# ndoll1998/lightgrad

Hardware: AMD Instinct MI355X
Metric: mnist_mlp_train_steps_per_sec_batch1024_per_gpu (higher is better)
Workload: dtype f32; 1 GPU; mnist_mlp_784x512x10_bias_batch1024_mse_adabelief_lr1e-3 (fwd+bwd+allreduce+optimizer); batch_per_gpu=1024, global_batch=1024, parallelism=dp1, optimizer_kernel=fused, input_requires_grad=True, dispatch=hipGraph replay (python tape captured once; 13 consecutive steps per graph), steps_per_graph=13, device=AMD Instinct (gfx950), compute_units=256, clock_mhz=2400

## Files before the change

### lightgrad_amd/csrc/gemm.hip

```cpp
#include "common.h"
#include "gelu_common.h"
#include "adam_common.h"
#include "tail_jobs.h"
#include "mse_finalize.h"
#include "head_fwd_body.h"
#include <cstdlib>
#include <cstring>
#include <type_traits>

namespace lg {

typedef float f32x16 __attribute__((ext_vector_type(16)));
typedef unsigned int u32x4 __attribute__((ext_vector_type(4)));
typedef float f32x4 __attribute__((ext_vector_type(4)));

#ifndef LG_SMALL_PD
#define LG_SMALL_PD 2
#endif
constexpr int kSmallTilePrefetch = LG_SMALL_PD;
#ifndef LG_WAVE_PRIVATE_PD
#define LG_WAVE_PRIVATE_PD 1
#endif
constexpr int kWavePrivatePrefetch = LG_WAVE_PRIVATE_PD;

struct FastDiv {
    uint32_t m, s;
    __device__ __forceinline__ int div(int n) const { return int((uint64_t(uint32_t(n)) * m) >> s); }
};
static FastDiv make_fastdiv(int64_t d) {
    if (d < 1) d = 1;
    uint32_t l = 0;
    while ((int64_t(1) << l) < d) ++l;
    FastDiv f;
    f.m = uint32_t((uint64_t(1) << (31 + l)) / uint64_t(d) + 1);
    f.s = 31 + l;
    return f;
}

struct GemmArgs {
    const float* A;
    const float* B;
    float*       C;
    int64_t M, N, K;
    int64_t lda, ldb, ldc;
    int64_t sA, sB, sC;
    int64_t sA2, sB2, sC2;
    int     batch_inner;
    int     tiles_m, tiles_n;
    int     nwg;
    int     accumulate;
    const float* bias;
    const float* addend;
    int64_t      ldadd;
    int     group_m;
    int     k_slices;
    int64_t k_per_slice;
    float*  W;
    int*    tickets;
    float*  rowsum;
    int     rowsum_accumulate;
    FastDiv div_per_batch, div_slices, div_gspan, div_group, div_last_group, div_batch_inner;
    int     k_tail;
    short   relu_a, relu_b;
    int     act;
    float*  aux;
    int     multi;
    int64_t boff[3], coff[3], biasoff[3];
    int     seg_k, seg_steps;
    int64_t seg_jump[2];
    const AdamPlan* adam_c;
    const AdamPlan* adam_r;
#ifdef LG_GEMM_TIMELINE
    unsigned long long* tl;
#endif
};

// ... 52 lines not shown
    constexpr int BM = 64, BN = 32, BK = 32, WM = 2, WN = 1, KG = 2, XT = 0;
    constexpr bool AKC = true, BKC = true, VA = true, VB = true;
    __shared__ __attribute__((aligned(16))) float lds[gemm_lds_floats<BM, BN, BK, AKC, BKC, KG>()];
    if (int(blockIdx.x) < g.nwg) {
        int* const signal_tickets = c.tickets;
        const int signal_stride = c.stride, signal_per_row = c.per_row;
#define LG_TILE_OWNS_LDS 0
#define LG_TILE_BID int(blockIdx.x)
#undef LG_TILE_SIGNAL
#define LG_TILE_SIGNAL 1
#include "gemm_tile_body.inc"
#undef LG_TILE_SIGNAL
#undef LG_TILE_BID
#undef LG_TILE_OWNS_LDS
    } else {
        const HeadFwd& a = c.h;
        const int tid = threadIdx.x, lane = tid & 63, wave = tid >> 6;
        const int wn = a.outs * a.hidden;
        for (int i = tid * 4; i < wn; i += 1024) *reinterpret_cast<float4*>(lds + i) = *reinterpret_cast<const float4*>(a.w + i);
        const int64_t row0 = int64_t(int(blockIdx.x) - g.nwg) * 4;
        int* const ticket = c.tickets + int(row0 / BM) * c.stride;
        const int64_t block_rows = a.rows - (row0 / BM) * BM < BM ? a.rows - (row0 / BM) * BM : BM;
        const int readers = int((block_rows + 3) / 4);
        int* const flag = ticket + 16;
        int* const done = ticket + 17;
        __shared__ int seen;
        if (tid == 0) {
            int ok = 1;
            const unsigned long long t0 = wall_clock64();
            while (__hip_atomic_load(flag, __ATOMIC_RELAXED, __HIP_MEMORY_SCOPE_AGENT) == 0) {
                __builtin_amdgcn_s_sleep(2);
                if (wall_clock64() - t0 > 200000000ull) {
                    __hip_atomic_fetch_or(c.status, LG_STATUS_HANDOFF_TIMEOUT, __ATOMIC_RELAXED, __HIP_MEMORY_SCOPE_SYSTEM);
                    ok = 0;
                    break;
                }
            }
            seen = ok;
        }
        __syncthreads();
        __builtin_amdgcn_fence(__ATOMIC_ACQUIRE, "wavefront");
        const int64_t row = row0 + wave;
        if (row < a.rows) head_fwd_row<OMAX, true>(a, lds, row, lane);
        if (tid == 0 && seen) {
            if (__hip_atomic_fetch_add(done, 1, __ATOMIC_RELAXED, __HIP_MEMORY_SCOPE_AGENT) == readers - 1) {
                __hip_atomic_store(done, 0, __ATOMIC_RELAXED, __HIP_MEMORY_SCOPE_AGENT);
                __hip_atomic_store(flag, 0, __ATOMIC_RELAXED, __HIP_MEMORY_SCOPE_AGENT);
            }
        }
    }
}

template <int PD, bool SECOND_BKC = false>
__global__ void __launch_bounds__(256) sgemm_pair_wgrad_xgrad(GemmArgs first, GemmArgs second) {
    constexpr int L1 = gemm_lds_floats<64, 64, 32, false, false, 1>(), L2 = gemm_lds_floats<64, 64, 32, true, SECOND_BKC, 1>();
    __shared__ __attribute__((aligned(16))) float lds[L1 > L2 ? L1 : L2];
    constexpr int BM = 64, BN = 64, BK = 32, WM = 2, WN = 2, KG = 1, XT = 0;
    constexpr bool VA = true, VB = true;
#define LG_TILE_OWNS_LDS 0
    if (int(blockIdx.x) < first.nwg) {
        constexpr bool AKC = false, BKC = false;
        const GemmArgs& g = first;
#define LG_TILE_BID int(blockIdx.x)
#include "gemm_tile_body.inc"
#undef LG_TILE_BID
    } else {
        constexpr bool AKC = true, BKC = SECOND_BKC;
        const GemmArgs& g = second;
#define LG_TILE_BID (int(blockIdx.x) - first.nwg)
#include "gemm_tile_body.inc"
#undef LG_TILE_BID
    }
#undef LG_TILE_OWNS_LDS
}

int lg_mse_finalize_job(const float* row_loss, int64_t rows, float inv_n, float* loss);
struct PairFirsts { GemmArgs w[2]; };
struct LossJob {
    const float* row_loss;
    float*       loss;
    int64_t      rows;
    float        inv_n;
};
template <int PD>
__global__ void __launch_bounds__(256) sgemm_triple_wgrad2_xgrad(PairFirsts firsts, GemmArgs second, LossJob job) {
    constexpr int L1 = gemm_lds_floats<64, 64, 32, false, false, 1>(), L2 = gemm_lds_floats<64, 64, 32, true, false, 1>();
    __shared__ __attribute__((aligned(16))) float lds[L1 > L2 ? L1 : L2];
    constexpr int BM = 64, BN = 64, BK = 32, WM = 2, WN = 2, KG = 1, XT = 0;
    constexpr bool VA = true, VB = true;
#define LG_TILE_OWNS_LDS 0
    const int n0w = firsts.w[0].nwg, n1w = firsts.w[1].nwg;
    if (int(blockIdx.x) < n0w + n1w) {
        constexpr bool AKC = false, BKC = false;
        const int which = int(blockIdx.x) >= n0w ? 1 : 0;
        const GemmArgs g = firsts.w[which];
#define LG_TILE_BID (int(blockIdx.x) - (which ? n0w : 0))
#include "gemm_tile_body.inc"
#undef LG_TILE_BID
    } else if (int(blockIdx.x) < n0w + n1w + second.nwg) {
        constexpr bool AKC = true, BKC = false;
        const GemmArgs& g = second;
#define LG_TILE_BID (int(blockIdx.x) - n0w - n1w)
#include "gemm_tile_body.inc"
#undef LG_TILE_BID
    } else {
        finalize_loss(job.row_loss, job.rows, job.inv_n, job.loss, lds);
    }
#undef LG_TILE_OWNS_LDS
}

constexpr int kGroupMax = 14;
struct GroupProduct {
    const float* A;
    const float* B;
    float*       C;
    float*       W;
    int*         tickets;
    float*       rowsum;
    int64_t      M, N, K, lda, ldb, ldc, k_per_slice;
    int          tiles_m, tiles_n, nwg, accumulate, group_m, k_slices, rowsum_accumulate, k_tail;
    FastDiv      div_per_batch, div_slices, div_gspan, div_group, div_last_group, div_batch_inner;
};
static GroupProduct pack_product(const GemmArgs& g) {
    return GroupProduct{g.A, g.B, g.C, g.W, g.tickets, g.rowsum, g.M, g.N, g.K, g.lda, g.ldb, g.ldc, g.k_per_slice,
                        g.tiles_m, g.tiles_n, g.nwg, g.accumulate, g.group_m, g.k_slices, g.rowsum_accumulate, g.k_tail,
                        g.div_per_batch, g.div_slices, g.div_gspan, g.div_group, g.div_last_group, g.div_batch_inner};
}
__device__ __forceinline__ GemmArgs unpack_product(const GroupProduct& p) {
    GemmArgs g{};
    g.A = p.A; g.B = p.B; g.C = p.C; g.W = p.W; g.tickets = p.tickets; g.rowsum = p.rowsum;
    g.M = p.M; g.N = p.N; g.K = p.K; g.lda = p.lda; g.ldb = p.ldb; g.ldc = p.ldc; g.k_per_slice = p.k_per_slice;
    g.tiles_m = p.tiles_m; g.tiles_n = p.tiles_n; g.nwg = p.nwg; g.accumulate = p.accumulate; g.group_m = p.group_m;
    g.k_slices = p.k_slices; g.rowsum_accumulate = p.rowsum_accumulate; g.k_tail = p.k_tail;
    g.div_per_batch = p.div_per_batch; g.div_slices = p.div_slices; g.div_gspan = p.div_gspan; g.div_group = p.div_group;
    g.div_last_group = p.div_last_group; g.div_batch_inner = p.div_batch_inner;
    g.batch_inner = 1;
    return g;
}

struct GemmGroup {
    GroupProduct p[kGroupMax];
    int      first[kGroupMax + 1];
    int      count;
    const float* cs_in;
    float*       cs_out;
    int64_t      cs_rows, cs_cols, cs_ld;
    int          cs_accumulate, cs_wgs;
    int          tail_wgs;
    TailGroup    tail;
};

static_assert(sizeof(GemmGroup) <= 4096, "the group travels as kernel arguments");

template <int PD>
__global__ void __launch_bounds__(256) sgemm_group_wgrad(GemmGroup grp) {
    __shared__ __attribute__((aligned(16))) float lds[gemm_lds_floats<64, 64, 32, false, false, 1>()];
    constexpr int BM = 64, BN = 64, BK = 32, WM = 2, WN = 2, KG = 1, XT = 0;
    constexpr bool VA = true, VB = true, AKC = false, BKC = false;
    if (int(blockIdx.x) < grp.cs_wgs) {
        const int q = threadIdx.x >> 6, cl = threadIdx.x & 63;
// ... 14 lines not shown
            grp.cs_out[col] = grp.cs_accumulate ? grp.cs_out[col] + v : v;
        }
        return;
    }
    const int bid = int(blockIdx.x) - grp.cs_wgs;
    if (bid >= grp.first[grp.count]) {
        tail_group_body(grp.tail, bid - grp.first[grp.count]);
        return;
    }
    int which = 0;
    while (which + 1 < grp.count && bid >= grp.first[which + 1]) ++which;
    const GemmArgs g = unpack_product(grp.p[which]);
#define LG_TILE_OWNS_LDS 0
#define LG_TILE_BID (bid - grp.first[which])
#include "gemm_tile_body.inc"
#undef LG_TILE_BID
#undef LG_TILE_OWNS_LDS
}

static thread_local int32_t g_gemm_plan[8] = {-1, 0, 0, 0, 0, 0, 0, 0};

template <int BM, int BN, int BK, int WM, int WN, bool AKC, bool BKC, int KG>
static bool launch_layout(const GemmArgs& g, bool va, bool vb) {
    dim3 grid(g.nwg), block(WM * WN * KG * 64);
    hipStream_t s = rt().stream;
    constexpr int PD = (BM * BN <= 64 * 64) ? kSmallTilePrefetch : 2;
    static_assert(BM * BN < 256 * 256 || PD <= 2, "a third K-tile in flight does not fit the 256x256 tile's 128 registers: ring registers would spill while their loads are in flight");
    if constexpr (kWavePrivateTile<BM, BN, WM, WN, KG> && AKC && BKC) {
        static const char* kloop_env = getenv("LG_GEMM_KLOOP");
        if (va && vb && !(kloop_env && strcmp(kloop_env, "coop") == 0)) {
            constexpr int WPD = kWavePrivatePrefetch;
            if (g.multi) hipLaunchKernelGGL((sgemm_mfma<BM, BN, BK, WM, WN, true, true, true, true, WPD, KG, 1, true>), grid, block, 0, s, g);
            else         hipLaunchKernelGGL((sgemm_mfma<BM, BN, BK, WM, WN, true, true, true, true, WPD, KG, 0, true>), grid, block, 0, s, g);
            return true;
        }
    }
    if constexpr (kHasExtras<BM, BN>) {
        if constexpr (AKC && BKC)  { if (g.multi) { hipLaunchKernelGGL((sgemm_mfma<BM, BN, BK, WM, WN, AKC, BKC, true, true, PD, KG, 1>), grid, block, 0, s, g); return false; } }
        if constexpr (AKC && !BKC) { if (g.seg_k) { hipLaunchKernelGGL((sgemm_mfma<BM, BN, BK, WM, WN, AKC, BKC, true, true, PD, KG, 2>), grid, block, 0, s, g); return false; } }
    }
    if constexpr (!kHasExtras<BM, BN>) {
        hipLaunchKernelGGL((sgemm_mfma<BM, BN, BK, WM, WN, AKC, BKC, true, true, PD, KG>), grid, block, 0, s, g);
        return false;
    }
    if (va && vb)  hipLaunchKernelGGL((sgemm_mfma<BM, BN, BK, WM, WN, AKC, BKC, true, true, PD, KG>), grid, block, 0, s, g);
    else if (va)   hipLaunchKernelGGL((sgemm_mfma<BM, BN, BK, WM, WN, AKC, BKC, true, false, 1, KG>), grid, block, 0, s, g);
    else if (vb)   hipLaunchKernelGGL((sgemm_mfma<BM, BN, BK, WM, WN, AKC, BKC, false, true, 1, KG>), grid, block, 0, s, g);
    else           hipLaunchKernelGGL((sgemm_mfma<BM, BN, BK, WM, WN, AKC, BKC, false, false, 1, KG>), grid, block, 0, s, g);
    return false;
}

#ifdef LG_GEMM_TIMELINE
static void lg_debug_timeline_state(unsigned long long* buf, int nwg, int slices, int tiles);
#endif
struct PairState {
    int      active = 0;
    int      count = 0;
    bool     second_bkc = false;
    GemmArgs args[3];
    bool     is_s[3] = {false, false, false};
    int64_t  batch[3] = {1, 1, 1};
    int64_t  tiles = 0;
    LossJob  job{};
};
static PairState& pair_state() { static PairState p; return p; }

static void pair_launch_single(const GemmArgs& g, bool is_s) {
    dim3 grid(g.nwg), block(256);
    constexpr int PD = kSmallTilePrefetch;
    if (!is_s) hipLaunchKernelGGL((sgemm_mfma<64, 64, 32, 2, 2, false, false, true, true, PD, 1>), grid, block, 0, rt().stream, g);
    else if (pair_state().second_bkc) hipLaunchKernelGGL((sgemm_mfma<64, 64, 32, 2, 2, true, true, true, true, PD, 1>), grid, block, 0, rt().stream, g);
    else           hipLaunchKernelGGL((sgemm_mfma<64, 64, 32, 2, 2, true, false, true, true, PD, 1>), grid, block, 0, rt().stream, g);
}

static int pair_retune(GemmArgs& g, int64_t others_nwg) {
    const int64_t tiles = int64_t(g.tiles_m) * g.tiles_n;
    static const char* pair_slices_env = getenv("LG_GEMM_PAIR_SLICES");
    if (pair_slices_env || g.nwg != tiles * g.k_slices || g.seg_k || tiles >= 256 || g.K < 128) return LG_OK;
    constexpr int BK = 32, BM = 64, BN = 64;
    const double cus = rt().compute_units > 0 ? rt().compute_units : 256;
    const int64_t k_tiles = (g.K + BK - 1) / BK;
    int64_t best_sl = g.k_slices;
    double best = 1e30;
    for (int64_t sl = 1; sl <= 64 && (sl == 1 || sl * 2 <= k_tiles); ++sl) {
        const double per_cu = double(tiles * sl + others_nwg) / cus;
        const double c = per_cu > 1.0 ? double(int64_t(per_cu + 0.999)) : 1.0;
        const double cost = double((k_tiles + sl - 1) / sl) * (c <= 1.0 ? 0.68 : 0.43 * c + 0.17) + (sl > 1 ? 1.8 + 0.85 * double(sl) : 0.0);
        if (cost < best) { best = cost; best_sl = sl; }
    }
    int64_t k_per_slice = ((g.K + best_sl - 1) / best_sl + BK - 1) / BK * BK;
    best_sl = (g.K + k_per_slice - 1) / k_per_slice;
    if (best_sl == g.k_slices) return LG_OK;
    if (g.W) { const int rc = lg_free(g.W); g.W = nullptr; if (rc != LG_OK) return rc; }
    g.k_per_slice = k_per_slice;
    g.k_slices = int(best_sl);
    g.nwg = int(tiles * best_sl);
    g.div_slices = make_fastdiv(best_sl);
    if (best_sl > 1) {
        const int rc = lg_malloc(reinterpret_cast<void**>(&g.W), size_t(tiles * best_sl) * BM * BN * sizeof(float));
        if (rc != LG_OK) return rc;
    }
    return LG_OK;
}

static int pair_flush(bool keep_collecting) {
    PairState& P = pair_state();
    int rc = LG_OK;
    bool job_done = false;
    if (P.count == 3) {
        rc = pair_retune(P.args[1], int64_t(P.args[0].nwg) + P.args[2].nwg);
        if (rc != LG_OK) { P.count = 0; return rc; }
        PairFirsts firsts;
        firsts.w[0] = P.args[0];
        firsts.w[1] = P.args[1];
        const int spare = P.job.loss ? 1 : 0;
        hipLaunchKernelGGL((sgemm_triple_wgrad2_xgrad<kSmallTilePrefetch>), dim3(P.args[0].nwg + P.args[1].nwg + P.args[2].nwg + spare), dim3(256), 0,
                           rt().stream, firsts, P.args[2], P.job);
        job_done = true;
    } else if (P.count == 2 && P.is_s[1]) {
        rc = pair_retune(P.args[0], P.args[1].nwg);
        if (rc != LG_OK) { P.count = 0; return rc; }
#ifdef LG_GEMM_TIMELINE
        if (P.args[0].tl) {
            (void)hipMemsetAsync(P.args[0].tl, 0, size_t(P.args[0].nwg + P.args[1].nwg) * 64, rt().stream);
            lg_debug_timeline_state(P.args[0].tl, P.args[0].nwg + P.args[1].nwg, P.args[0].k_slices * 100 + P.args[1].k_slices, P.args[0].nwg);
        }
#endif
        if (P.second_bkc)
            hipLaunchKernelGGL((sgemm_pair_wgrad_xgrad<kSmallTilePrefetch, true>), dim3(P.args[0].nwg + P.args[1].nwg), dim3(256), 0, rt().stream,
                               P.args[0], P.args[1]);
        else
            hipLaunchKernelGGL((sgemm_pair_wgrad_xgrad<kSmallTilePrefetch, false>), dim3(P.args[0].nwg + P.args[1].nwg), dim3(256), 0, rt().stream,
                               P.args[0], P.args[1]);
    } else {
        for (int i = 0; i < P.count; ++i) pair_launch_single(P.args[i], P.is_s[i]);
    }
    for (int i = 0; i < P.count; ++i)
        if (P.args[i].W) { const int r = lg_free(P.args[i].W); if (r != LG_OK) rc = r; }
    P.count = 0;
    P.tiles = 0;
    if (job_done) P.job = LossJob{};
    if (!keep_collecting && P.active) P.active = 2;
    return rc;
}

struct WriteSpan { uintptr_t lo, hi; };
static WriteSpan product_c_span(const GemmArgs& g, int64_t batch) {
    const int64_t outer = batch / g.batch_inner;
    int64_t lo = 0, hi = (g.M - 1) * g.ldc + g.N;
    const int64_t reach[2] = {(outer - 1) * g.sC, int64_t(g.batch_inner - 1) * g.sC2};
    for (int64_t r : reach) { if (r < 0) lo += r; else hi += r; }
    const uintptr_t base = reinterpret_cast<uintptr_t>(g.C);
    return WriteSpan{base + uintptr_t(lo * 4), base + uintptr_t(hi * 4)};
}
static bool spans_meet(WriteSpan a, WriteSpan b) { return a.lo < b.hi && b.lo < a.hi; }
static bool products_write_alike(const GemmArgs& a, int64_t batch_a, const GemmArgs& b, int64_t batch_b) {
    const WriteSpan none{0, 0};
    const WriteSpan ca = product_c_span(a, batch_a), cb = product_c_span(b, batch_b);
    const WriteSpan ra = a.rowsum ? WriteSpan{reinterpret_cast<uintptr_t>(a.rowsum), reinterpret_cast<uintptr_t>(a.rowsum + a.M)} : none;
    const WriteSpan rb = b.rowsum ? WriteSpan{reinterpret_cast<uintptr_t>(b.rowsum), reinterpret_cast<uintptr_t>(b.rowsum + b.M)} : none;
    return spans_meet(ca, cb) || spans_meet(ca, rb) || spans_meet(ra, cb) || spans_meet(ra, rb);
}

static bool pair_try_defer(GemmArgs& g, bool akc, bool bkc, bool va, bool vb, int64_t batch) {
    PairState& P = pair_state();
    if (P.active != 1) return false;
    const int slot = P.count;
    for (int i = 0; i < slot; ++i)
        if (products_write_alike(P.args[i], P.batch[i], g, batch)) return false;
    const bool f_form = !akc && !bkc, s_form = akc;
    bool fits = slot < 3 && va && vb && batch >= 1;
    if (slot == 0)      fits = fits && f_form;
    else if (slot == 1) fits = fits && !P.is_s[0] && (f_form || s_form);
    else                fits = fits && !P.is_s[1] && s_form && !bkc && batch == 1 && !g.relu_a && !g.relu_b;
    if (slot == 1 && f_form) fits = fits && batch == 1 && P.args[0].nwg == int64_t(P.args[0].tiles_m) * P.args[0].tiles_n * P.args[0].k_slices;
    const int64_t tiles = int64_t(g.tiles_m) * g.tiles_n * batch;
    if (!fits || P.tiles + tiles > rt().n_tickets) return false;
    g.tickets = rt().tickets + P.tiles;
// ... 41 lines not shown
        bool ride = true;
        for (int i = 0; i < G.count; ++i) ride = ride && !ln_group_writes(G.queued[i].C) && !ln_group_writes(G.queued[i].rowsum);
        ride = ride && !ln_group_writes(G.grp.cs_wgs > 0 ? G.grp.cs_out : nullptr);
        G.grp.tail_wgs = 0;
        if (ride && tail_take(&G.grp.tail)) {
            G.grp.tail_wgs = G.grp.tail.first[G.grp.tail.ln.count + G.grp.tail.n_scatter];
        }
        hipLaunchKernelGGL((sgemm_group_wgrad<kSmallTilePrefetch>), dim3(G.grp.cs_wgs + G.grp.tail_wgs + G.grp.first[G.count]), dim3(256), 0, rt().stream, G.grp);
        if (G.grp.tail_wgs > 0) { const int r = tail_taken(); if (r != LG_OK) rc = r; }
    }
    for (int i = 0; i < G.count; ++i)
        if (G.queued[i].W) { const int r = lg_free(G.queued[i].W); if (r != LG_OK) rc = r; }
    G.count = 0;
    G.tiles = 0;
    G.grp.cs_wgs = 0;
    return rc;
}

static bool group_try_defer(GemmArgs& g, bool akc, bool bkc, bool va, bool vb, int64_t batch, int& rc) {
    GroupState& G = group_state();
    rc = LG_OK;
    if (G.active != 1 || pair_state().active) return false;
    const int64_t tiles = int64_t(g.tiles_m) * g.tiles_n;
    if (akc || bkc || !va || !vb || batch != 1 || tiles > kGroupTiles || g.relu_a || g.relu_b || g.multi || g.seg_k) return false;
    if (g.adam_c || g.adam_r) return false;
    bool clash = false;
    for (int i = 0; i < G.count; ++i)
        clash = clash || G.queued[i].C == g.C || (g.rowsum && G.queued[i].rowsum == g.rowsum);
    if (ln_group_writes(g.C) || ln_group_writes(g.rowsum)) {
        rc = gemm_group_flush_pending();
        if (rc != LG_OK) return false;
    } else if (clash || G.count == kGroupMax || G.tiles + tiles > tickets_group_end()) {
        rc = group_flush();
        if (rc != LG_OK) return false;
    }
    g.tickets = rt().tickets + G.tiles;
    G.tiles += tiles;
    G.queued[G.count] = g;
    G.count += 1;
    return true;
}

bool gemm_group_is_open() { return group_state().active == 1; }

int gemm_group_flush_pending() {
    if (pair_state().count) { const int prc = pair_flush(true); if (prc != LG_OK) return prc; }
    const int rc = group_flush();
    const int rc2 = ln_group_flush_pending();
    return rc != LG_OK ? rc : rc2;
}

#ifdef LG_GEMM_TIMELINE
static unsigned long long* g_tl_buf = nullptr;
static int g_tl_nwg = 0, g_tl_slices = 0, g_tl_tiles = 0;
static void lg_debug_timeline_state(unsigned long long* buf, int nwg, int slices, int tiles) {
    g_tl_buf = buf; g_tl_nwg = nwg; g_tl_slices = slices; g_tl_tiles = tiles;
}
#endif

template <int BM, int BN, int BK, int WM, int WN, int KG = 1>
static int launch_config(const GemmArgs& base, bool akc, bool bkc, bool va, bool vb, int64_t batch) {
    GemmArgs g = base;
    g.tiles_m = int((g.M + BM - 1) / BM);
    g.tiles_n = int((g.N + (g.rowsum ? 1 : 0) + BN - 1) / BN);
    const int64_t tiles = int64_t(g.tiles_m) * g.tiles_n * batch;
    int64_t slices = 1;
    if (kCanSplitK<BM, BN, KG> && tiles < 256 && g.K >= 4 * BK) {
        const double cus = rt().compute_units > 0 ? rt().compute_units : 256;
        const double t_iter = BM * BN >= 128 * 128 ? 2.4 : (BM * BN >= 64 * 64 ? 0.65 : 0.45);
        const int64_t k_tiles = (g.K + BK - 1) / BK;
        double best = 1e30;
        for (int64_t sl = 1; sl <= 64 && sl * 2 <= k_tiles; ++sl) {
            const double per_cu = double(tiles * sl) / cus;
            const double kt = double((k_tiles + sl - 1) / sl);
            double cost;
            if (BM * BN == 64 * 64) {
                const double c = per_cu > 1.0 ? double(int64_t(per_cu + 0.999)) : 1.0;
                cost = kt * (c <= 1.0 ? 0.68 : 0.43 * c + 0.17) + (sl > 1 ? 1.8 + 0.85 * double(sl) : 0.0);
            } else {
                cost = kt * t_iter * (per_cu > 1.0 ? per_cu : 1.0) + (sl > 1 ? 2.0 + 0.6 * double(sl) : 0.0);
            }
            if (cost < best) { best = cost; slices = sl; }
        }
    }
    static const char* slices_env = getenv("LG_GEMM_SLICES");
    if (kCanSplitK<BM, BN, KG> && slices_env && atoi(slices_env) >= 1) slices = atoi(slices_env);
    static const char* pair_slices_env = getenv("LG_GEMM_PAIR_SLICES");
    if (kCanSplitK<BM, BN, KG> && pair_slices_env && pair_state().active == 1) {
        int sv[3] = {0, 0, 0};
        const int got = sscanf(pair_slices_env, "%d,%d,%d", &sv[0], &sv[1], &sv[2]);
        if (got >= 2) { const int c = pair_state().count; const int v = c < got ? sv[c] : sv[got - 1]; if (v >= 1) slices = v; }
    }
    if (g.seg_k) { slices = 1; g.seg_steps = g.seg_k / (BK * KG); }
    g.k_per_slice = ((g.K + slices - 1) / slices + BK - 1) / BK * BK;
    slices = (g.K + g.k_per_slice - 1) / g.k_per_slice;
    g.k_slices = int(slices);
    g.nwg = int(tiles * slices);
    g.div_per_batch = make_fastdiv(int64_t(g.tiles_m) * g.tiles_n);
    g.div_slices = make_fastdiv(slices);
    g.div_gspan = make_fastdiv(int64_t(g.group_m) * g.tiles_n);
    g.div_group = make_fastdiv(g.group_m);
    g.div_last_group = make_fastdiv(g.tiles_m % g.group_m ? g.tiles_m % g.group_m : g.group_m);
    g.div_batch_inner = make_fastdiv(g.batch_inner);
    g.W = nullptr;
    g.tickets = rt().tickets;
#ifdef LG_GEMM_TIMELINE
    {
        static unsigned long long* tl_buf = nullptr;
        if (!tl_buf) (void)hipMalloc(reinterpret_cast<void**>(&tl_buf), size_t(1) << 22);
        g.tl = (tl_buf && size_t(g.nwg) * 64 <= (size_t(1) << 22)) ? tl_buf : nullptr;
// ... 257 lines not shown
    LG_ARG(hidden % 4 == 0 && aligned16(pre) && aligned16(w2) && outs * hidden * 4 <= 64 * 1024,
           "lg_gemm_bias_head_fwd_f32: hidden a multiple of 4, pre and w2 16-byte aligned, w2 within 64 KiB (lg_head_fwd_f32's conditions)");
    HeadChain c{};
    c.h.x = pre; c.h.w = w2; c.h.bias = b2; c.h.target = target; c.h.y = y; c.h.err = err; c.h.row_loss = row_loss; c.h.gpre = gpre; c.h.dx = dx;
    c.h.rows = rows; c.h.ldx = hidden; c.h.hidden = int(hidden); c.h.outs = int(outs); c.h.relu = relu;
    c.tickets = rt().tickets + kChainTicketBase;
    c.stride = kChainTicketStride;
    c.status = rt().status_dev;
    constexpr int kLdsFloats = gemm_lds_floats<64, 32, 32, true, true, 2>();
    const bool can_chain = chain != 0 && hidden <= 1024 && outs * hidden <= kLdsFloats && rows <= int64_t(kChainRowBlocks) * 64
                           && kChainTicketBase + kChainRowBlocks * kChainTicketStride <= tickets_group_end() && aligned16(dx) && aligned16(gpre);
    if (can_chain) pending_chain() = &c;
    const int rc = gemm_impl(0, 1, rows, hidden, d_in, x, ldx, 0, w1, ldw1, 0, pre, hidden, 0, 1, 0, b1);
    const bool chained = can_chain && pending_chain() == nullptr;
    pending_chain() = nullptr;
    if (rc != LG_OK) return rc;
    if (launches) *launches = chained ? 1 : 2;
    if (chained) return LG_OK;
    return lg_head_fwd_grad_f32(pre, hidden, relu, w2, b2, target, y, err, row_loss, dx, gpre, rows, hidden, outs);
}

extern "C" int lg_gemm_batched2_f32(int transA, int transB, int64_t M, int64_t N, int64_t K,
                                    const float* A, int64_t lda, int64_t strideA_outer, int64_t strideA_inner,
                                    const float* B, int64_t ldb, int64_t strideB_outer, int64_t strideB_inner,
                                    float* C, int64_t ldc, int64_t strideC_outer, int64_t strideC_inner,
                                    int64_t batch_outer, int64_t batch_inner, int accumulate) {
    LG_ARG(batch_outer >= 0 && batch_inner >= 0 && batch_inner < (int64_t(1) << 30), "lg_gemm_batched2_f32: bad batch extents");
    if (batch_outer == 0 || batch_inner == 0) return LG_OK;
    return gemm_impl(transA, transB, M, N, K, A, lda, strideA_outer, B, ldb, strideB_outer, C, ldc, strideC_outer,
                     batch_outer * batch_inner, accumulate, nullptr, nullptr, 0, batch_inner, strideA_inner, strideB_inner, strideC_inner);
}

extern "C" int lg_gemm_fused_f32(int transA, int transB, int64_t M, int64_t N, int64_t K,
                                 const float* A, int64_t lda, const float* B, int64_t ldb, float* C, int64_t ldc,
                                 int accumulate, const float* bias, float* rowsum, int rowsum_accumulate,
                                 int relu_a, int relu_b) {
    LG_ARG(!(bias && rowsum), "lg_gemm_fused_f32: bias and rowsum exclude each other");
    LG_ARG(!(bias && accumulate), "lg_gemm_fused_f32: bias and accumulate exclude each other");
    return gemm_impl(transA, transB, M, N, K, A, lda, 0, B, ldb, 0, C, ldc, 0, 1, accumulate, bias, rowsum, rowsum_accumulate,
                     1, 0, 0, 0, relu_a, relu_b);
}

#ifdef LG_GEMM_TIMELINE
extern "C" int lg_debug_gemm_timeline(unsigned long long* host, int max_wgs, int* nwg, int* slices, int* tiles) {
    LG_REQUIRE_INIT();
    LG_HIP(hipStreamSynchronize(rt().stream));
    const int n = lg::g_tl_nwg < max_wgs ? lg::g_tl_nwg : max_wgs;
    if (lg::g_tl_buf && n > 0) LG_HIP(hipMemcpy(host, lg::g_tl_buf, size_t(n) * 64, hipMemcpyDeviceToHost));
    *nwg = n; *slices = lg::g_tl_slices; *tiles = lg::g_tl_tiles;
    return LG_OK;
}
#endif

extern "C" int lg_gemm_pair_begin(void) {
    LG_REQUIRE_INIT();
    PairState& P = lg::pair_state();
    LG_ARG(P.active == 0, "lg_gemm_pair_begin: a pair bracket is already open");
    P.active = 1;
    P.count = 0;
    return LG_OK;
}

extern "C" int lg_gemm_pair_end(void) {
    LG_REQUIRE_INIT();
    PairState& P = lg::pair_state();
    LG_ARG(P.active != 0, "lg_gemm_pair_end: no pair bracket is open");
    int rc = lg::pair_flush(true);
    P.active = 0;
    if (P.job.loss) {
        const int r = lg::lg_mse_finalize_job(P.job.row_loss, P.job.rows, P.job.inv_n, P.job.loss);
        P.job = lg::LossJob{};
        if (r != LG_OK) rc = r;
    }
    if (rc != LG_OK) return rc;
    LG_CHECK_LAUNCH();
    return LG_OK;
}

extern "C" int lg_gemm_pair_hold(void) {
    LG_REQUIRE_INIT();
    PairState& P = lg::pair_state();
    LG_ARG(P.active == 1 || P.active == 2, "lg_gemm_pair_hold: no pair bracket is open");
    if (P.active == 1) P.active = 3;
    return LG_OK;
}

extern "C" int lg_gemm_pair_resume(void) {
    LG_REQUIRE_INIT();
    PairState& P = lg::pair_state();
    LG_ARG(P.active != 0, "lg_gemm_pair_resume: no pair bracket is open");
    if (P.active == 3) P.active = 1;
    return LG_OK;
}

extern "C" int lg_gemm_pair_mse_loss(const float* row_loss, int64_t rows, int64_t n, float* loss) {
    LG_REQUIRE_INIT();
    PairState& P = lg::pair_state();
    LG_ARG(P.active != 0, "lg_gemm_pair_mse_loss: no pair bracket is open");
    LG_ARG(row_loss && loss && rows > 0 && n > 0, "lg_gemm_pair_mse_loss: bad arguments");
    LG_ARG(P.job.loss == nullptr, "lg_gemm_pair_mse_loss: the bracket already carries a loss");
    P.job.row_loss = row_loss; P.job.loss = loss; P.job.rows = rows;
    P.job.inv_n = float(1.0 / double(n));
    return LG_OK;
}

extern "C" int lg_gemm_group_begin(void) {
// ... 92 lines not shown
```

### lightgrad_amd/csrc/gemm_tile_body.inc

```
#ifndef LG_TILE_SIGNAL
#define LG_TILE_SIGNAL 0
#endif
#ifndef LG_TILE_WAVE_PRIVATE
#define LG_TILE_WAVE_PRIVATE false
#endif
    constexpr bool WPK = LG_TILE_WAVE_PRIVATE;
    static_assert(!WPK || (KG > 1 && WM * WN == 1 && BM == 32 && BN == 32 && AKC && BKC && VA && VB && XT != 2 && !LG_TILE_SIGNAL), "wave-private K loop: one wave per K-group, NT form");
    constexpr int NT = WM * WN * KG * 64;
    constexpr int NTS = WPK ? 64 : NT;
    constexpr int BKS = WPK ? BK : BK * KG;
    constexpr int TM = BM / WM / 32, TN = BN / WN / 32;
    static_assert(TM >= 1 && TN >= 1 && BK % 16 == 0 && (KG == 1 || KG == 2 || KG == 4), "tile config");
    constexpr bool AG = kGatherStaging<BM, BN, AKC>, BG = kGatherStaging<BM, BN, BKC>;
    static_assert((!AG || VA) && (!BG || VB), "gather staging replaces the float4 form");
    constexpr bool ALK = AKC || AG, BLK = BKC || BG;
    constexpr int A_PITCH = ALK ? BKS + 4 : BM;
    constexpr int B_PITCH = BLK ? BKS + 4 : BN;
    constexpr int A_TILE = ALK ? BM * A_PITCH : BKS * A_PITCH;
    constexpr int B_TILE = BLK ? BN * B_PITCH : BKS * B_PITCH;
    constexpr int A_ELEMS = BM * BKS / NTS, B_ELEMS = BN * BKS / NTS;
    static_assert(A_ELEMS % 4 == 0 && B_ELEMS % 4 == 0, "staging must divide into float4");

    static_assert(WPK || 2 * (A_TILE + B_TILE) == gemm_lds_floats<BM, BN, BK, AKC, BKC, KG>(), "LDS size");
    static_assert(!(AG || BG) || TM * TN > 1, "gather staging: the multi-accumulator loop only");
#if LG_TILE_OWNS_LDS
    __shared__ __attribute__((aligned(16))) float lds[gemm_lds_floats<BM, BN, BK, AKC, BKC, KG>()];
#endif
    constexpr int BUF = A_TILE + B_TILE;

    const int tid = threadIdx.x;
    const int lane = tid & 63, wave = tid >> 6;
    const int kg = WPK ? __builtin_amdgcn_readfirstlane(wave) : wave / (WM * WN), wl = wave % (WM * WN);
    const int wm = wl / WN, wn = wl % WN;
    const int kofs = WPK ? 0 : kg * BK;
    const int stid = WPK ? lane : tid;
    float* const ldsw = WPK ? lds + kg * BUF : lds;
    const int r = lane & 31, h = lane >> 5;
    LG_TL(0);

    const int id = xcd_remap(LG_TILE_BID, g.nwg);
    const int per_batch = g.tiles_m * g.tiles_n;
    const int bs = g.div_per_batch.div(id);
    const int batch = g.div_slices.div(bs), slice = bs - batch * g.k_slices;
    const int t = id - bs * per_batch;
    const int GROUP_M = g.group_m;
    const int gspan = GROUP_M * g.tiles_n;
    const int group = g.div_gspan.div(t);
    const int first_m = group * GROUP_M, in_group = t - group * gspan;
    const bool last_group = g.tiles_m - first_m < GROUP_M;
    const int gsize = last_group ? g.tiles_m - first_m : GROUP_M;
    const int tn = last_group ? g.div_last_group.div(in_group) : g.div_group.div(in_group);
    const int tm = first_m + (in_group - tn * gsize);
    const int64_t m0 = int64_t(tm) * BM, n0 = int64_t(tn) * BN;
    const int b_outer = g.div_batch_inner.div(batch), b_inner = batch - b_outer * g.batch_inner;
    const float* __restrict__ A = g.A + int64_t(b_outer) * g.sA + int64_t(b_inner) * g.sA2;
    const float* Bp = g.B + int64_t(b_outer) * g.sB + int64_t(b_inner) * g.sB2;
    float* Cp = g.C + int64_t(b_outer) * g.sC + int64_t(b_inner) * g.sC2;
// ... 237 lines not shown
#pragma unroll
    for (int i = 0; i < TM; ++i)
#pragma unroll
        for (int j = 0; j < TN; ++j)
#pragma unroll
            for (int e = 0; e < 16; ++e) acc[i][j][e] = 0.f;

    auto compute_tile = [&](int buf, int kb_begin, int kb_end) {
        const float* a = lds + buf * BUF + (ALK ? (wm * TM * 32 + r) * A_PITCH + 4 * h + kofs : (4 * h + kofs) * A_PITCH + wm * TM * 32 + r);
        const float* b = lds + buf * BUF + A_TILE + (BLK ? (wn * TN * 32 + r) * B_PITCH + 4 * h + kofs : (4 * h + kofs) * B_PITCH + wn * TN * 32 + r);
#pragma unroll
        for (int kb = kb_begin; kb < kb_end; kb += 8) {
            float fa[TM][4], fb[TN][4];
#pragma unroll
            for (int i = 0; i < TM; ++i) {
                if constexpr (ALK) {
                    const float4 v = *reinterpret_cast<const float4*>(a + i * 32 * A_PITCH + kb);
                    fa[i][0] = v.x; fa[i][1] = v.y; fa[i][2] = v.z; fa[i][3] = v.w;
                } else {
#pragma unroll
                    for (int s = 0; s < 4; ++s) fa[i][s] = a[(kb + s) * A_PITCH + i * 32];
                }
            }
#pragma unroll
            for (int j = 0; j < TN; ++j) {
                if constexpr (BLK) {
                    const float4 v = *reinterpret_cast<const float4*>(b + j * 32 * B_PITCH + kb);
                    fb[j][0] = v.x; fb[j][1] = v.y; fb[j][2] = v.z; fb[j][3] = v.w;
                } else {
#pragma unroll
                    for (int s = 0; s < 4; ++s) fb[j][s] = b[(kb + s) * B_PITCH + j * 32];
                }
            }
#pragma unroll
            for (int s = 0; s < 4; ++s)
#pragma unroll
                for (int i = 0; i < TM; ++i)
#pragma unroll
                    for (int j = 0; j < TN; ++j)
                        acc[i][j] = __builtin_amdgcn_mfma_f32_32x32x2f32(fa[i][s], fb[j][s], acc[i][j], 0, 0, 0);
        }
    };

#pragma unroll
    for (int u = 0; u < PD; ++u)
        if (u < nkt) load_tile(u);
    if constexpr (!WPK) {
        const int younger = nkt - 1 < PD - 1 ? nkt - 1 : PD - 1;
        wait_tile(0, younger);
        store_tile(0, 0);
        __syncthreads();
    }
    LG_TL(1);
    if constexpr (WPK) {
        static_assert(BK == 16, "one K-step is two k-blocks of 8");
        float fa[2][4], fb[2][4];
        auto read_half = [&](int half, int set) {
            const float4 va = *reinterpret_cast<const float4*>(ldsw + r * A_PITCH + 4 * h + half * 8);
            const float4 vb = *reinterpret_cast<const float4*>(ldsw + A_TILE + r * B_PITCH + 4 * h + half * 8);
            fa[set][0] = va.x; fa[set][1] = va.y; fa[set][2] = va.z; fa[set][3] = va.w;
            fb[set][0] = vb.x; fb[set][1] = vb.y; fb[set][2] = vb.z; fb[set][3] = vb.w;
        };
        auto mfma_part = [&](int set, int e0, int e1) {
#pragma unroll
            for (int e = e0; e < e1; ++e)
                acc[0][0] = __builtin_amdgcn_mfma_f32_32x32x2f32(fa[set][e], fb[set][e], acc[0][0], 0, 0, 0);
        };
        auto advance = [&](int t, int slot) {
            const int younger = (nkt < t + PD ? nkt : t + PD) - (t + 1);
            wait_tile(slot, younger);
            store_tile(0, slot);
            if (t + PD < nkt) load_tile(slot);
        };
        if (nkt > 0) {
            advance(0, 0);
            read_half(0, 0);
        }
        for (int kt0 = 0; kt0 < nkt; kt0 += PD) {
#pragma unroll
            for (int u = 0; u < PD; ++u) {
                const int kt = kt0 + u;
                if (kt < nkt) {
                    read_half(1, 1);
                    mfma_part(0, 0, 4);
                    __builtin_amdgcn_sched_barrier(0);
                    if (kt + 1 < nkt) advance(kt + 1, (u + 1) % PD);
                    __builtin_amdgcn_sched_barrier(0);
                    mfma_part(1, 0, 1);
                    __builtin_amdgcn_sched_barrier(0);
                    if (kt + 1 < nkt) read_half(0, 0);
                    mfma_part(1, 1, 4);
                }
            }
        }
    } else if constexpr (TM * TN == 1) {
        constexpr int HG = BK / 16;
        float fa[2][HG][4], fb[2][HG][4];
        auto read_half = [&](int buf, int half, int slot) {
            const float* a = lds + buf * BUF + (AKC ? (wm * 32 + r) * A_PITCH + 4 * h + kofs : (4 * h + kofs) * A_PITCH + wm * 32 + r);
            const float* b = lds + buf * BUF + A_TILE + (BKC ? (wn * 32 + r) * B_PITCH + 4 * h + kofs : (4 * h + kofs) * B_PITCH + wn * 32 + r);
#pragma unroll
            for (int q = 0; q < HG; ++q) {
                const int kb = half * (BK / 2) + q * 8;
                if constexpr (AKC) {
                    const float4 v = *reinterpret_cast<const float4*>(a + kb);
                    fa[slot][q][0] = v.x; fa[slot][q][1] = v.y; fa[slot][q][2] = v.z; fa[slot][q][3] = v.w;
// ... 18 lines not shown
                    acc[0][0] = __builtin_amdgcn_mfma_f32_32x32x2f32(fa[slot][q][e], fb[slot][q][e], acc[0][0], 0, 0, 0);
        };
        auto mfma_half = [&](int slot) { mfma_part(slot, 0, HG); };
        constexpr int HQ = HG > 1 ? HG / 2 : HG;
        read_half(0, 0, 0);
        for (int kt0 = 0; kt0 < nkt; kt0 += PD) {
#pragma unroll
            for (int u = 0; u < PD; ++u) {
                const int kt = kt0 + u;
                if (kt < nkt) {
                    const int cur = kt & 1;
                    if (PD == 1 && kt + 1 < nkt) load_tile(0);
                    read_half(cur, 1, 1);
                    mfma_part(0, 0, HQ);
                    __builtin_amdgcn_sched_barrier(0);
                    if (kt + 1 < nkt) {
                        int younger = nkt - (kt + 2);
                        if (younger > PD - 2) younger = PD - 2;
                        wait_tile((u + 1) % PD, PD == 1 ? 0 : (younger < 0 ? 0 : younger));
                        store_tile(cur ^ 1, (u + 1) % PD);
                    }
                    if (PD > 1 && kt + PD < nkt) load_tile(u);
                    __builtin_amdgcn_sched_barrier(0);
                    mfma_part(0, HQ, HG);
                    __syncthreads();
                    if (kt + 1 < nkt) read_half(cur ^ 1, 0, 0);
                    mfma_half(1);
                }
            }
        }
    } else {
        for (int kt0 = 0; kt0 < nkt; kt0 += PD) {
    #pragma unroll
            for (int u = 0; u < PD; ++u) {
                const int kt = kt0 + u;
                if (kt < nkt) {
                    const int cur = kt & 1;
                    if (PD == 1 && kt + 1 < nkt) load_tile(0);
                    compute_tile(cur, 0, BK / 2);
                    if (kt + 1 < nkt) {
                        int younger = nkt - (kt + 2);
                        if (younger > PD - 2) younger = PD - 2;
                        wait_tile((u + 1) % PD, PD == 1 ? 0 : (younger < 0 ? 0 : younger));
                        store_tile(cur ^ 1, (u + 1) % PD);
                    }
                    if (PD > 1 && kt + PD < nkt) load_tile(u);
                    compute_tile(cur, BK / 2, BK);
                    __syncthreads();
                }
            }
        }
    }

    LG_TL(2);
    if constexpr (KG > 1) {
        constexpr int GROUP_FLOATS = WM * WN * TM * TN * 16 * 64;
        static_assert(WPK || (KG - 1) * GROUP_FLOATS <= 2 * (A_TILE + B_TILE), "the K-group exchange must fit the staging buffers");
        static_assert(!WPK || KG * BUF + (KG - 1) * GROUP_FLOATS <= gemm_lds_floats<BM, BN, BK, AKC, BKC, KG>(), "staging regions + exchange");
        float* x = lds + (WPK ? KG * BUF : 0) + (wl * TM * TN * 16) * 64 + lane;
        if (kg >= 1) {
#pragma unroll
            for (int i = 0; i < TM; ++i)
#pragma unroll
                for (int j = 0; j < TN; ++j)
#pragma unroll
                    for (int e = 0; e < 16; ++e) x[(kg - 1) * GROUP_FLOATS + ((i * TN + j) * 16 + e) * 64] = acc[i][j][e];
        }
        __syncthreads();
        if (kg >= 1) return;
#pragma unroll
        for (int gq = 0; gq < KG - 1; ++gq)
#pragma unroll
            for (int i = 0; i < TM; ++i)
#pragma unroll
                for (int j = 0; j < TN; ++j)
#pragma unroll
                    for (int e = 0; e < 16; ++e) acc[i][j][e] += x[gq * GROUP_FLOATS + ((i * TN + j) * 16 + e) * 64];
    }
    [[maybe_unused]] AdamScalars adam_cs_c, adam_cs_r;
    [[maybe_unused]] int64_t adam_done_c = 0, adam_done_r = 0;
    if constexpr (kCanAdam<BM, BN, KG>) {
        if (g.adam_c) adam_cs_c = adam_plan_scalars(g.adam_c, adam_done_c);
        if (g.adam_r) adam_cs_r = adam_plan_scalars(g.adam_r, adam_done_r);
    }
    if constexpr (kCanSplitK<BM, BN, KG>) if (g.k_slices > 1) {
        constexpr int SC1 = 16;
        constexpr int TILE_BYTES = BM * BN * 4;
        char* slab0 = reinterpret_cast<char*>(g.W) + (int64_t(batch) * g.k_slices * per_batch + t) * int64_t(TILE_BYTES);
        const int64_t slice_stride = int64_t(per_batch) * TILE_BYTES;
        {
            const auto mine = __builtin_amdgcn_make_buffer_rsrc(slab0 + slice * slice_stride, 0, TILE_BYTES, 0x00020000);
#pragma unroll
            for (int i = 0; i < TM; ++i)
#pragma unroll
                for (int j = 0; j < TN; ++j)
#pragma unroll
                    for (int q = 0; q < 4; ++q) {
                        u32x4 v;
#pragma unroll
                        for (int e = 0; e < 4; ++e) v[e] = __float_as_uint(acc[i][j][4 * q + e]);
                        __builtin_amdgcn_raw_buffer_store_b128(v, mine, (((i * TN + j) * 4 + q) * NT + tid) * 16, 0, SC1);
                    }
        }
        asm volatile("s_waitcnt vmcnt(0)" ::: "memory");
        __syncthreads();
        LG_TL(3);
        int* arrived_last = reinterpret_cast<int*>(lds);
        if (tid == 0) {
            int* ticket = g.tickets + batch * per_batch + t;
            const int order = __hip_atomic_fetch_add(ticket, 1, __ATOMIC_RELAXED, __HIP_MEMORY_SCOPE_AGENT);
            const int last = order == g.k_slices - 1;
            if (last) __hip_atomic_store(ticket, 0, __ATOMIC_RELAXED, __HIP_MEMORY_SCOPE_AGENT);
            *arrived_last = last;
        }
        __syncthreads();
        LG_TL(4);
        if (!*arrived_last) return;
        __builtin_amdgcn_fence(__ATOMIC_ACQUIRE, "wavefront");
        constexpr int CH = TM * TN >= 4 ? 1 : (TM * TN == 2 ? 2 : 4);
        for (int s0 = 0; s0 < g.k_slices; s0 += CH) {
            u32x4 v[CH][TM * TN * 4];
#pragma unroll
            for (int c = 0; c < CH; ++c) {
                const int sl = s0 + c < g.k_slices ? s0 + c : s0;
                const auto src = __builtin_amdgcn_make_buffer_rsrc(slab0 + sl * slice_stride, 0, TILE_BYTES, 0x00020000);
#pragma unroll
                for (int f = 0; f < TM * TN * 4; ++f) v[c][f] = __builtin_amdgcn_raw_buffer_load_b128(src, (f * NT + tid) * 16, 0, SC1);
            }
#pragma unroll
            for (int c = 0; c < CH; ++c) {
                const bool live = s0 + c < g.k_slices, first = s0 + c == 0;
#pragma unroll
                for (int i = 0; i < TM; ++i)
#pragma unroll
                    for (int j = 0; j < TN; ++j)
#pragma unroll
                        for (int e = 0; e < 16; ++e) {
                            const float w = __uint_as_float(v[c][(i * TN + j) * 4 + e / 4][e % 4]);
                            acc[i][j][e] = first ? w : (live ? acc[i][j][e] + w : acc[i][j][e]);
                        }
            }
        }
    }

    LG_TL(5);
    int etid = threadIdx.x;
    asm volatile("" : "+v"(etid));
    const int ewl = (etid >> 6) % (WM * WN), er = etid & 31, eh = (etid >> 5) & 1;
    const int ewm = ewl / WN, ewn = ewl % WN;
#pragma unroll
    for (int i = 0; i < TM; ++i) {
#pragma unroll
        for (int j = 0; j < TN; ++j) {
            const int64_t col = n0 + (ewn * TN + j) * 32 + er;
            const int64_t row0 = m0 + (ewm * TM + i) * 32 + 4 * eh;
            const bool vcol = has_virtual && col == g.N;
            if (col < g.N || vcol) {
                float bv = 0.f;
                if constexpr (kHasExtras<BM, BN>) bv = (bias && !vcol) ? bias_ahead[j] : 0.f;
                else                              bv = bias ? bias[col] : 0.f;
                float* const dst = vcol ? g.rowsum : C + col;
                const int64_t dstride = vcol ? 1 : ldc;
                const float* const addend = vcol ? nullptr : g.addend;
                const bool acc_flag = vcol ? g.rowsum_accumulate != 0 : (accumulate != 0 || addend != nullptr);
                const float* const old_src = addend ? addend + col : dst;
                const int64_t old_stride = addend ? g.ldadd : dstride;
                float val[16];
#pragma unroll
                for (int e = 0; e < 16; ++e) val[e] = bias ? acc[i][j][e] + bv : acc[i][j][e];
                if (acc_flag) {
                    float old[16];
#pragma unroll
                    for (int e = 0; e < 16; ++e) {
// ... 95 lines not shown
```

Baseline: 21210 steps/s.

## Fold last-arriver split-K reduction into registers and add occupancy hint to pair kernels

In the split-K last-arriver epilogue of the pair/triple backward GEMM kernels, the last-arriving slice now keeps its own partial sum in registers. When the slice count is small, it loads only the other slices' partials in one pass and adds them in slice order, instead of reloading every slice including its own. This removes one round trip of tile loads and the loop over chunks. The pair and triple kernels also get a minimum-waves-per-EU launch bound, which constrains register use to raise occupancy and may cause spills. An optional s_setprio for the xgrad tiles, off by default, and timeline debug role bookkeeping are added.

```diff
diff --git a/lightgrad_amd/csrc/gemm.hip b/lightgrad_amd/csrc/gemm.hip
--- a/lightgrad_amd/csrc/gemm.hip
+++ b/lightgrad_amd/csrc/gemm.hip
@@ -22,6 +22,15 @@
 #define LG_WAVE_PRIVATE_PD 1
 #endif
 constexpr int kWavePrivatePrefetch = LG_WAVE_PRIVATE_PD;
+#ifndef LG_DX_PRIO
+#define LG_DX_PRIO 0
+#endif
+#ifndef LG_FOLD_ONE_TRIP
+#define LG_FOLD_ONE_TRIP 1
+#endif
+#ifndef LG_SHARED_WAVES
+#define LG_SHARED_WAVES 4
+#endif
 
 struct FastDiv {
     uint32_t m, s;
@@ -180,11 +189,13 @@
 }
 
 template <int PD, bool SECOND_BKC = false>
-__global__ void __launch_bounds__(256) sgemm_pair_wgrad_xgrad(GemmArgs first, GemmArgs second) {
+__global__ void __launch_bounds__(256, LG_SHARED_WAVES) sgemm_pair_wgrad_xgrad(GemmArgs first, GemmArgs second) {
     constexpr int L1 = gemm_lds_floats<64, 64, 32, false, false, 1>(), L2 = gemm_lds_floats<64, 64, 32, true, SECOND_BKC, 1>();
     __shared__ __attribute__((aligned(16))) float lds[L1 > L2 ? L1 : L2];
     constexpr int BM = 64, BN = 64, BK = 32, WM = 2, WN = 2, KG = 1, XT = 0;
     constexpr bool VA = true, VB = true;
+#undef LG_TILE_FOLD_ONE_TRIP
+#define LG_TILE_FOLD_ONE_TRIP LG_FOLD_ONE_TRIP
 #define LG_TILE_OWNS_LDS 0
     if (int(blockIdx.x) < first.nwg) {
         constexpr bool AKC = false, BKC = false;
@@ -196,9 +207,15 @@
         constexpr bool AKC = true, BKC = SECOND_BKC;
         const GemmArgs& g = second;
 #define LG_TILE_BID (int(blockIdx.x) - first.nwg)
+#undef LG_TILE_PRIO
+#define LG_TILE_PRIO LG_DX_PRIO
 #include "gemm_tile_body.inc"
+#undef LG_TILE_PRIO
+#define LG_TILE_PRIO 0
 #undef LG_TILE_BID
     }
+#undef LG_TILE_FOLD_ONE_TRIP
+#define LG_TILE_FOLD_ONE_TRIP 0
 #undef LG_TILE_OWNS_LDS
 }
 
@@ -211,11 +228,13 @@
     float        inv_n;
 };
 template <int PD>
-__global__ void __launch_bounds__(256) sgemm_triple_wgrad2_xgrad(PairFirsts firsts, GemmArgs second, LossJob job) {
+__global__ void __launch_bounds__(256, LG_SHARED_WAVES) sgemm_triple_wgrad2_xgrad(PairFirsts firsts, GemmArgs second, LossJob job) {
     constexpr int L1 = gemm_lds_floats<64, 64, 32, false, false, 1>(), L2 = gemm_lds_floats<64, 64, 32, true, false, 1>();
     __shared__ __attribute__((aligned(16))) float lds[L1 > L2 ? L1 : L2];
     constexpr int BM = 64, BN = 64, BK = 32, WM = 2, WN = 2, KG = 1, XT = 0;
     constexpr bool VA = true, VB = true;
+#undef LG_TILE_FOLD_ONE_TRIP
+#define LG_TILE_FOLD_ONE_TRIP LG_FOLD_ONE_TRIP
 #define LG_TILE_OWNS_LDS 0
     const int n0w = firsts.w[0].nwg, n1w = firsts.w[1].nwg;
     if (int(blockIdx.x) < n0w + n1w) {
@@ -229,11 +248,17 @@
         constexpr bool AKC = true, BKC = false;
         const GemmArgs& g = second;
 #define LG_TILE_BID (int(blockIdx.x) - n0w - n1w)
+#undef LG_TILE_PRIO
+#define LG_TILE_PRIO LG_DX_PRIO
 #include "gemm_tile_body.inc"
+#undef LG_TILE_PRIO
+#define LG_TILE_PRIO 0
 #undef LG_TILE_BID
     } else {
         finalize_loss(job.row_loss, job.rows, job.inv_n, job.loss, lds);
     }
+#undef LG_TILE_FOLD_ONE_TRIP
+#define LG_TILE_FOLD_ONE_TRIP 0
 #undef LG_TILE_OWNS_LDS
 }
 
@@ -354,6 +379,7 @@
 
 #ifdef LG_GEMM_TIMELINE
 static void lg_debug_timeline_state(unsigned long long* buf, int nwg, int slices, int tiles);
+static void lg_debug_timeline_roles(int a, int b, int c);
 #endif
 struct PairState {
     int      active = 0;
@@ -412,6 +438,16 @@
     if (P.count == 3) {
         rc = pair_retune(P.args[1], int64_t(P.args[0].nwg) + P.args[2].nwg);
         if (rc != LG_OK) { P.count = 0; return rc; }
+#ifdef LG_GEMM_TIMELINE
+        if (P.args[0].tl) {
+            const int all = P.args[0].nwg + P.args[1].nwg + P.args[2].nwg;
+            unsigned long long* const tl = size_t(all) * 64 <= (size_t(1) << 22) ? P.args[0].tl : nullptr;
+            for (int i = 0; i < 3; ++i) P.args[i].tl = tl;
+            if (tl) (void)hipMemsetAsync(tl, 0, size_t(all) * 64, rt().stream);
+            lg_debug_timeline_state(tl, all, P.args[1].k_slices * 100 + P.args[2].k_slices, P.args[1].nwg);
+            lg_debug_timeline_roles(P.args[0].nwg, P.args[1].nwg, P.args[2].nwg);
+        }
+#endif
         PairFirsts firsts;
         firsts.w[0] = P.args[0];
         firsts.w[1] = P.args[1];
@@ -426,6 +462,7 @@
         if (P.args[0].tl) {
             (void)hipMemsetAsync(P.args[0].tl, 0, size_t(P.args[0].nwg + P.args[1].nwg) * 64, rt().stream);
             lg_debug_timeline_state(P.args[0].tl, P.args[0].nwg + P.args[1].nwg, P.args[0].k_slices * 100 + P.args[1].k_slices, P.args[0].nwg);
+            lg_debug_timeline_roles(P.args[0].nwg, P.args[1].nwg, 0);
         }
 #endif
         if (P.second_bkc)
@@ -573,10 +610,12 @@
 
 #ifdef LG_GEMM_TIMELINE
 static unsigned long long* g_tl_buf = nullptr;
-static int g_tl_nwg = 0, g_tl_slices = 0, g_tl_tiles = 0;
+static int g_tl_nwg = 0, g_tl_slices = 0, g_tl_tiles = 0, g_tl_roles[3] = {0, 0, 0};
 static void lg_debug_timeline_state(unsigned long long* buf, int nwg, int slices, int tiles) {
     g_tl_buf = buf; g_tl_nwg = nwg; g_tl_slices = slices; g_tl_tiles = tiles;
-}
+    g_tl_roles[0] = nwg; g_tl_roles[1] = g_tl_roles[2] = 0;
+}
+static void lg_debug_timeline_roles(int a, int b, int c) { g_tl_roles[0] = a; g_tl_roles[1] = b; g_tl_roles[2] = c; }
 #endif
 
 template <int BM, int BN, int BK, int WM, int WN, int KG = 1>
@@ -940,6 +979,13 @@
 }
 #endif
 
+#ifdef LG_GEMM_TIMELINE
+extern "C" int lg_debug_gemm_timeline_roles(int* roles) {
+    for (int i = 0; i < 3; ++i) roles[i] = lg::g_tl_roles[i];
+    return LG_OK;
+}
+#endif
+
 extern "C" int lg_gemm_pair_begin(void) {
     LG_REQUIRE_INIT();
     PairState& P = lg::pair_state();
diff --git a/lightgrad_amd/csrc/gemm_tile_body.inc b/lightgrad_amd/csrc/gemm_tile_body.inc
--- a/lightgrad_amd/csrc/gemm_tile_body.inc
+++ b/lightgrad_amd/csrc/gemm_tile_body.inc
@@ -3,6 +3,12 @@
 #endif
 #ifndef LG_TILE_WAVE_PRIVATE
 #define LG_TILE_WAVE_PRIVATE false
+#endif
+#ifndef LG_TILE_PRIO
+#define LG_TILE_PRIO 0
+#endif
+#ifndef LG_TILE_FOLD_ONE_TRIP
+#define LG_TILE_FOLD_ONE_TRIP 0
 #endif
     constexpr bool WPK = LG_TILE_WAVE_PRIVATE;
     static_assert(!WPK || (KG > 1 && WM * WN == 1 && BM == 32 && BN == 32 && AKC && BKC && VA && VB && XT != 2 && !LG_TILE_SIGNAL), "wave-private K loop: one wave per K-group, NT form");
@@ -346,6 +352,9 @@
         __syncthreads();
     }
     LG_TL(1);
+#if LG_TILE_PRIO > 0
+    __builtin_amdgcn_s_setprio(LG_TILE_PRIO);
+#endif
     if constexpr (WPK) {
         static_assert(BK == 16, "one K-step is two k-blocks of 8");
         float fa[2][4], fb[2][4];
@@ -470,6 +479,9 @@
         }
     }
 
+#if LG_TILE_PRIO > 0
+    __builtin_amdgcn_s_setprio(0);
+#endif
     LG_TL(2);
     if constexpr (KG > 1) {
         constexpr int GROUP_FLOATS = WM * WN * TM * TN * 16 * 64;
@@ -536,7 +548,58 @@
         if (!*arrived_last) return;
         __builtin_amdgcn_fence(__ATOMIC_ACQUIRE, "wavefront");
         constexpr int CH = TM * TN >= 4 ? 1 : (TM * TN == 2 ? 2 : 4);
-        for (int s0 = 0; s0 < g.k_slices; s0 += CH) {
+        if (LG_TILE_FOLD_ONE_TRIP && g.k_slices <= CH + 1) {
+            const int others = g.k_slices - 1;
+            u32x4 v[CH][TM * TN * 4];
+#pragma unroll
+            for (int c = 0; c < CH; ++c) {
+                const int sl = c < slice ? c : c + 1;
+                const auto src = __builtin_amdgcn_make_buffer_rsrc(slab0 + sl * slice_stride, 0, c < others ? TILE_BYTES : 0, 0x00020000);
+#pragma unroll
+                for (int f = 0; f < TM * TN * 4; ++f) v[c][f] = __builtin_amdgcn_raw_buffer_load_b128(src, (f * NT + tid) * 16, 0, SC1);
+            }
+            auto W = [&](int c, int i, int j, int e) { return __uint_as_float(v[c][(i * TN + j) * 4 + e / 4][e % 4]); };
+            auto add_from = [&](int c0) {
+#pragma unroll
+                for (int c = c0; c < CH; ++c)
+                    if (c >= slice && c < others) {
+#pragma unroll
+                        for (int i = 0; i < TM; ++i)
+#pragma unroll
+                            for (int j = 0; j < TN; ++j)
+#pragma unroll
+                                for (int e = 0; e < 16; ++e) acc[i][j][e] = acc[i][j][e] + W(c, i, j, e);
+                    }
+            };
+            if (slice == 0) {
+                add_from(0);
+            } else {
+                f32x16 below[TM][TN];
+#pragma unroll
+                for (int i = 0; i < TM; ++i)
+#pragma unroll
+                    for (int j = 0; j < TN; ++j)
+#pragma unroll
+                        for (int e = 0; e < 16; ++e) below[i][j][e] = W(0, i, j, e);
+#pragma unroll
+                for (int c = 1; c < CH; ++c)
+                    if (c < slice) {
+#pragma unroll
+                        for (int i = 0; i < TM; ++i)
+#pragma unroll
+                            for (int j = 0; j < TN; ++j)
+#pragma unroll
+                                for (int e = 0; e < 16; ++e) below[i][j][e] = below[i][j][e] + W(c, i, j, e);
+                    }
+#pragma unroll
+                for (int i = 0; i < TM; ++i)
+#pragma unroll
+                    for (int j = 0; j < TN; ++j)
+#pragma unroll
+                        for (int e = 0; e < 16; ++e) acc[i][j][e] = below[i][j][e] + acc[i][j][e];
+                add_from(1);
+            }
+        } else for (int s0 = 0; s0 < g.k_slices; s0 += CH) {
             u32x4 v[CH][TM * TN * 4];
 #pragma unroll
             for (int c = 0; c < CH; ++c) {
```

Result: no change. 21380 steps/s (median of 6 runs) (+0.8%).
